# TopHillRobotics/quadruped-robot

Hardware: AMD Instinct MI355X
Metric: MPC+WBC control ticks/s (batched robots) (higher is better)
Workload: dtype f32 assembly / f64 QP+WBC

## Files before the change

### quadruped-robot_amd/csrc/qr_mpc_kernel.hip

```cpp
#include <hip/hip_runtime.h>
#include <type_traits>
#include "qr_device_types.h"
#include "qr_wave_helpers.h"
#include "qr_kernels.h"

namespace qrgpu {

#ifdef QR_TIMELINE
#define QR_TRACE(rid_, bits_) do { if (P.tl && P.solved) atomicOr((unsigned long long *)(P.tl + QR_TL_TRACE + (P.solved_epoch & 15u) * 1024 + ((rid_) & 1023)), (unsigned long long)(bits_) | ((unsigned long long)(P.solved_epoch & 15u) << 32) | (1ull << 40)); } while (0)
#define QR_P_TL P.tl
#define QR_P_FTIME P.ftime
#else
#define QR_TRACE(rid_, bits_) do { } while (0)
#define QR_P_TL ((long long *)nullptr)
#define QR_P_FTIME ((int *)nullptr)
#endif

#define QR_AS_THREADS 256
#define QR_RCP_PIVOT fast_rcp1
#define QR_REFRESH_EVERY 100
#ifdef QR_FLOPS_BUILD
#define qr_mpc_kernel qr_mpc_kernel_fl
#define mpc_solve_robot mpc_solve_robot_fl
#define QR_PFLOPS P.flops
// ... 487 lines not shown
                for (int r = r0; r < h; ++r) {
                    const bool onR = r >= iaR;
                    const float cR = ((float)r + bR) * dt2;
                    float gR = cR * a0R;
                    float tR = gR * w2q0;
                    gR = onR ? gR : 0.f; tR = onR ? tR : 0.f;
                    acc1 = __builtin_amdgcn_mfma_f32_16x16x4f32(tR, gR, acc1, 0, 0, 0);
                    const float hR = cR * a1R;
                    gR = (g < 2) ? hR : k1R; tR = (g < 2) ? hR * w2q1 : t1R;
                    gR = onR ? gR : 0.f; tR = onR ? tR : 0.f;
                    acc1 = __builtin_amdgcn_mfma_f32_16x16x4f32(tR, gR, acc1, 0, 0, 0);
                    gR = onR ? k2R : 0.f; tR = onR ? t2R : 0.f;
                    acc1 = __builtin_amdgcn_mfma_f32_16x16x4f32(tR, gR, acc1, 0, 0, 0);
                }
            } else {
                for (int r = r0; r < h; ++r) {
                    const bool onR = r >= iaR, onC = r >= iaC;
                    const float rf = (float)r;
                    const float cR = (rf + bR) * dt2, cC = (rf + bC) * dt2;
                    float gR = cR * a0R, gC = cC * a0C;
                    float tR = gR * w2q0, tC = gC * w2q0;
                    gR = onR ? gR : 0.f; tR = onR ? tR : 0.f; gC = onC ? gC : 0.f; tC = onC ? tC : 0.f;
                    acc1 = __builtin_amdgcn_mfma_f32_16x16x4f32(tR, gC, acc1, 0, 0, 0);
                    acc2 = __builtin_amdgcn_mfma_f32_16x16x4f32(gR, tC, acc2, 0, 0, 0);
                    const float hR = cR * a1R, hC = cC * a1C;
                    gR = (g < 2) ? hR : k1R; tR = (g < 2) ? hR * w2q1 : t1R;
                    gC = (g < 2) ? hC : k1C; tC = (g < 2) ? hC * w2q1 : t1C;
                    gR = onR ? gR : 0.f; tR = onR ? tR : 0.f; gC = onC ? gC : 0.f; tC = onC ? tC : 0.f;
                    acc1 = __builtin_amdgcn_mfma_f32_16x16x4f32(tR, gC, acc1, 0, 0, 0);
                    acc2 = __builtin_amdgcn_mfma_f32_16x16x4f32(gR, tC, acc2, 0, 0, 0);
                    gR = onR ? k2R : 0.f; tR = onR ? t2R : 0.f; gC = onC ? k2C : 0.f; tC = onC ? t2C : 0.f;
                    acc1 = __builtin_amdgcn_mfma_f32_16x16x4f32(tR, gC, acc1, 0, 0, 0);
                    acc2 = __builtin_amdgcn_mfma_f32_16x16x4f32(gR, tC, acc2, 0, 0, 0);
                }
            }
            float *buf = Hs + 256 * (diag ? 2 * NOD + R : 2 * (((R * (R - 1)) >> 1) + Cc));
#pragma unroll
            for (int reg = 0; reg < 4; ++reg) buf[((4 * reg + g) ^ (Cc & 1)) * 16 + lc] = acc1[reg];
            if (!diag) {
#pragma unroll
                for (int reg = 0; reg < 4; ++reg) buf[256 + ((4 * reg + g) ^ (Cc & 1)) * 16 + lc] = acc2[reg];
            }
            if (Hd) {
                const int ec = 16 * Cc + lc;
#pragma unroll
                for (int reg = 0; reg < 4; ++reg) {
                    const int er = 16 * R + 4 * g + reg;
                    if (er < ns && ec < ns) {
                        const int aq = (er * 21846) >> 16, bq = (ec * 21846) >> 16;
                        const int xr_ = 3 * sLs[aq] + (er - 3 * aq), xc_ = 3 * sLs[bq] + (ec - 3 * bq);
                        Hd[(size_t)xr_ * NV + xc_] = acc1[reg] + ((er == ec) ? two_alpha : 0.f);
                        if (!diag) Hd[(size_t)xc_ * NV + xr_] = acc2[reg];
                    }
                }
            }
          }
        }
    }
    for (int e = tid - (NTHR - 128); e >= 0 && e < ns; e += 128) {
#pragma clang fp contract(off)
        const int ls = sLs[e / 3], j = e % 3, ia = ls >> 2, p = ls & 3;
        const float t0 = sT[9 * p + j], t1 = sT[9 * p + 3 + j], t2 = sT[9 * p + 6 + j];
        const float wg0 = 2.f * C.weights[0], wg1 = 2.f * C.weights[1], wg2 = 2.f * C.weights[2], wg3 = 2.f * C.weights[3 + j], wg9 = 2.f * C.weights[9 + j];
        const float u0 = (dt * sU[9 * p + j]) * (2.f * C.weights[6]), u1 = (dt * sU[9 * p + 3 + j]) * (2.f * C.weights[7]), u2 = (dt * sU[9 * p + 6 + j]) * (2.f * C.weights[8]);
        const float dw = dtm * wg9;
        float acc = 0.f;
        const float bA = 0.5f - (float)ia;
        for (int r = 0; r < h; ++r) {
            const float ca = ((float)r + bA) * dt2;
            const float *vr = sV + 13 * r;
            float a2 = acc;
            a2 = __builtin_fmaf((ca * t0) * wg0, vr[0], a2);
            a2 = __builtin_fmaf((ca * t1) * wg1, vr[1], a2);
            a2 = __builtin_fmaf((ca * t2) * wg2, vr[2], a2);
            a2 = __builtin_fmaf((ca * minv) * wg3, vr[3 + j], a2);
            a2 = __builtin_fmaf(u0, vr[6], a2);
            a2 = __builtin_fmaf(u1, vr[7], a2);
            a2 = __builtin_fmaf(u2, vr[8], a2);
            a2 = __builtin_fmaf(dw, vr[9 + j], a2);
            acc = (r >= ia) ? a2 : acc;
        }
        gl[e] = (double)acc;
        if (QR_DBGG) QR_DBGG[(size_t)rid * NV + 3 * ls + j] = acc;
    }
    for (int c = tid; c < 6 * nls; c += NTHR) sPos[c] = -1;
    QR_TS(2);

    Blk A[MAXB];
    QR_SYNC();
#pragma unroll
    for (int sl = 0; sl < MAXB; ++sl) {
        if (ba[sl] >= 0) {
            const int a = ba[sl], b = bb[sl];
            int rowb[3], rr[3], rp[3], Rx[3], colb[3], cc[3], cp[3], Cy[3];
#pragma unroll
            for (int i = 0; i < 3; ++i) {
                const int x = 3 * a + i, y = 3 * b + i;
                Rx[i] = x >> 4; rr[i] = x & 15; rp[i] = 4 * (rr[i] & 3) + (rr[i] >> 2); rowb[i] = 256 * Rx[i] * (Rx[i] - 1);
                Cy[i] = y >> 4; cc[i] = y & 15; cp[i] = 4 * (cc[i] & 3) + (cc[i] >> 2); colb[i] = 512 * Cy[i] + cc[i];
            }
            const int dbase = 512 * NOD;
#pragma unroll
            for (int i = 0; i < 3; ++i)
#pragma unroll
                for (int j = 0; j < 3; ++j) {
                    if (a == b && j > i) continue;
                    const bool od = Rx[i] != Cy[j];
                    const int dg = dbase + 256 * Rx[i], par = Cy[j] & 1;
                    const int a1 = od ? rowb[i] + colb[j] + 16 * (rp[i] ^ par) : dg + 16 * (rp[i] ^ par) + cc[j];
                    const int a2 = od ? a1 + 256 : dg + 16 * (cp[j] ^ par) + rr[i];
                    float v1 = Hs[a1], v2 = Hs[a2];
                    if (a == b && i == j) {
#pragma clang fp contract(off)
                        v1 = v1 + two_alpha; v2 = v1;
                    }
                    const double o = 0.5 * ((double)v1 + (double)v2);
                    A[sl].m[3 * i + j] = o;
                    if (a == b) A[sl].m[3 * j + i] = o;
                }
        }
    }
    QR_SYNC();
    if (NTHR > QR_AS_THREADS && tid >= QR_AS_THREADS && (tid & ~63) >= npairs) { if (PERSIST) QR_IDLE(); return; }
    {
        double *panel0 = Mb, *panel1 = Mb + NL * 9;
#define VS_STAMP(i) do { } while (0)
        auto write_panel = [&](int sl, int kk, double *pn) {
            if (bb[sl] == kk) {
                if (ba[sl] == kk) {
                    const double *Pk = A[sl].m;
                    const double p00 = Pk[0], p01 = 0.5 * (Pk[1] + Pk[3]), p02 = 0.5 * (Pk[2] + Pk[6]), p11 = Pk[4], p12 = 0.5 * (Pk[5] + Pk[7]), p22 = Pk[8];
                    const double c00 = p11 * p22 - p12 * p12, c01 = p02 * p12 - p01 * p22, c02 = p01 * p12 - p02 * p11;
                    const double c11 = p00 * p22 - p02 * p02, c12 = p01 * p02 - p00 * p12, c22 = p00 * p11 - p01 * p01;
                    const double det = p00 * c00 + p01 * c01 + p02 * c02;
                    if (!(det > 0.0) || !(p00 > 0.0)) sMisc[1] = 1;
                    const double id = QR_RCP_PIVOT(det);
                    double *d = pn + 9 * kk;
                    d[0] = c00 * id; d[1] = c01 * id; d[2] = c02 * id; d[4] = c11 * id; d[5] = c12 * id; d[8] = c22 * id;
                } else {
#pragma unroll
                    for (int i = 0; i < 9; ++i) pn[9 * ba[sl] + i] = A[sl].m[i];
                }
            } else if (ba[sl] == kk) {
#pragma unroll
                for (int i = 0; i < 3; ++i)
#pragma unroll
                    for (int j = 0; j < 3; ++j) pn[9 * bb[sl] + 3 * j + i] = A[sl].m[3 * i + j];
            }
        };
#pragma unroll
        for (int sl = 0; sl < MAXB; ++sl) write_panel(sl, 0, panel0);
        for (int k = 0; k < nls; ++k) {
            double *pan = (k & 1) ? panel1 : panel0, *pnext = (k & 1) ? panel0 : panel1;
            VS_STAMP(3);
            VS_STAMP(0);
            QR_SYNC();
            VS_STAMP(1);
            double Cx0[9], Cb0[9];
            {
                const int a0 = ba[0] < 0 ? 0 : ba[0], b0 = ba[0] < 0 ? 0 : bb[0];
                const double *Cx = pan + 9 * (a0 == k ? b0 : a0), *Cb = pan + 9 * b0;
#pragma unroll
                for (int i = 0; i < 9; ++i) { Cx0[i] = Cx[i]; Cb0[i] = Cb[i]; }
            }
            double Pi[9];
            {
                const double *Pk = pan + 9 * k;
                Pi[0] = Pk[0]; Pi[1] = Pk[1]; Pi[2] = Pk[2]; Pi[4] = Pk[4]; Pi[5] = Pk[5]; Pi[8] = Pk[8];
                Pi[3] = Pi[1]; Pi[6] = Pi[2]; Pi[7] = Pi[5];
            }
            VS_STAMP(2);
#pragma unroll
            for (int sl = 0; sl < MAXB; ++sl) {
                const int a = ba[sl], b = bb[sl];
                if (a < 0) continue;
                double Cxv[9], Cb[9];
                if (sl == 0) {
#pragma unroll
                    for (int i = 0; i < 9; ++i) { Cxv[i] = Cx0[i]; Cb[i] = Cb0[i]; }
                } else {
                    const double *Cxp = pan + 9 * (a == k ? b : a), *Cbp = pan + 9 * b;
#pragma unroll
                    for (int i = 0; i < 9; ++i) { Cxv[i] = Cxp[i]; Cb[i] = Cbp[i]; }
                }
                const double *Cx = Cxv;
                double D[9];
#pragma unroll
                for (int i = 0; i < 3; ++i)
#pragma unroll
                    for (int j = 0; j < 3; ++j) D[3 * i + j] = __builtin_fma(Cx[3 * i + 2], Pi[6 + j], __builtin_fma(Cx[3 * i + 1], Pi[3 + j], Cx[3 * i] * Pi[j]));
                if (a != k && b != k) {
#pragma unroll
                    for (int i = 0; i < 3; ++i)
#pragma unroll
                        for (int j = 0; j < 3; ++j)
                            A[sl].m[3 * i + j] = __builtin_fma(-D[3 * i + 2], Cb[3 * j + 2], __builtin_fma(-D[3 * i + 1], Cb[3 * j + 1], __builtin_fma(-D[3 * i], Cb[3 * j], A[sl].m[3 * i + j])));
                } else {
                    const bool tr = (a == k);
                    A[sl].m[0] = D[0]; A[sl].m[4] = D[4]; A[sl].m[8] = D[8];
                    A[sl].m[1] = tr ? D[3] : D[1]; A[sl].m[3] = tr ? D[1] : D[3];
                    A[sl].m[2] = tr ? D[6] : D[2]; A[sl].m[6] = tr ? D[2] : D[6];
                    A[sl].m[5] = tr ? D[7] : D[5]; A[sl].m[7] = tr ? D[5] : D[7];
                    if (a == k && b == k) {
#pragma unroll
                        for (int i = 0; i < 9; ++i) A[sl].m[i] = -Pi[i];
                    }
                }
                write_panel(sl, k + 1, pnext);
                __builtin_amdgcn_sched_barrier(0);
            }
        }
        QR_SYNC();
#pragma unroll
        for (int sl = 0; sl < MAXB; ++sl) {
            if (ba[sl] >= 0) {
                double *dst = Mb + (tri(ba[sl]) + bb[sl]) * 9;
#pragma unroll
                for (int i = 0; i < 9; ++i) dst[i] = -A[sl].m[i];
            }
        }
        QR_SYNC();
    }
    if (NTHR > QR_AS_THREADS && tid >= QR_AS_THREADS) { if (PERSIST) QR_IDLE(); return; }
    if (sMisc[1]) st |= QRGPU_ST_MPC_NOTSPD;
    QR_TS(3);
    if (QR_PFLOPS) {
        double steps = 0.0;
        for (int Rf = 0; Rf < NT; ++Rf) steps += (double)(2 * Rf + 1) * (double)(h - (sLs[(16 * Rf * 21846) >> 16] >> 2));
        fl_m32 = steps * 3.0 * 2048.0;
        fl_v32 = steps * 64.0 * 8.0;
        double gsteps = 0.0;
        for (int kf = 0; kf < nls; ++kf) gsteps += (double)(h - (sLs[kf] >> 2));
        fl_v32 += gsteps * 3.0 * 24.0;
        fl_sw = (double)nls * ((double)npairs * 99.0 + 40.0) + (double)nls * (double)nls * 15.0;
    }
    {
        const int wv = __builtin_amdgcn_readfirstlane(tid >> 6);
        const bool own = lane < nls;
        const int kme = own ? lane : 0;
        const double im = (double)(1.f / C.mu);
        const double fmaxk = own ? fmk[kme] : 0.0;
        const int tril = tri(lane);
        const double tol = 1e-9;
        const double INF = __builtin_inf();
        const bool big2 = BIG && qcap > 64;
        double *xr2 = xr2_in_floats ? (double *)sT : smem + (P.lds_bytes / 8 - 256);
        const int tril2 = tri(lane + 64);
        auto rd2 = [&](double v0, double v1, int j) { return j < 64 ? readlane_d(v0, j) : readlane_d(v1, j - 64); };
        int *sCtl = sMisc + 8;
        double *dd = xz;
        enum { F_FULL = 1, F_DROP = 2 };
        double x0 = 0.0, x1 = 0.0, x2 = 0.0;
        {
            double p0 = 0.0, p1 = 0.0, p2 = 0.0;
            if (own) {
                for (int kc = wv; kc < nls; kc += 4) {
                    Blk B; load_block(Mb, kme, kc, B);
                    const double g0 = gl[3 * kc], g1 = gl[3 * kc + 1], g2 = gl[3 * kc + 2];
                    p0 += B.m[0] * g0 + B.m[1] * g1 + B.m[2] * g2;
                    p1 += B.m[3] * g0 + B.m[4] * g1 + B.m[5] * g2;
                    p2 += B.m[6] * g0 + B.m[7] * g1 + B.m[8] * g2;
                }
                xz[wv * NV + 3 * kme] = p0; xz[wv * NV + 3 * kme + 1] = p1; xz[wv * NV + 3 * kme + 2] = p2;
            }
            if (wv == 0) for (int e = lane; e < 6 * nls; e += 64) sPos[e] = (short)-1;
            QR_SYNC();
            if (own) {
#pragma unroll
                for (int v = 0; v < 4; ++v) { x0 -= xz[v * NV + 3 * kme]; x1 -= xz[v * NV + 3 * kme + 1]; x2 -= xz[v * NV + 3 * kme + 2]; }
                if (wv == 0) { gl[3 * kme] = x0; gl[3 * kme + 1] = x1; gl[3 * kme + 2] = x2; }
            }
            QR_SYNC();
        }
        QR_TS(4);
        bool fastz = qW > 0;
        auto r_partial = [&](int q, double dq, double dq2) {
            if (BIG && q > 64) {
                const int i1 = (lane + 64 < q) ? lane + 64 : 0;
                double pa = 0.0, pb = 0.0;
                for (int j = wv; j < q; j += 4) {
                    const double dj = rd2(dq, dq2, j);
                    pa += Sinv[(j <= lane) ? tril + j : tri(j) + lane] * dj;
                    pb += Sinv[(j <= i1) ? tri(i1) + j : tri(j) + i1] * dj;
                }
                xr[wv * 64 + lane] = pa; xr2[wv * 64 + lane] = pb;
                return;
            }
            const int i0 = (lane < q) ? lane : 0;
            double pr = 0.0;
            int j = wv;
            for (; j + 12 < q; j += 16) {
                double sv[4], dj[4];
#pragma unroll
                for (int u = 0; u < 4; ++u) { const int jj = j + 4 * u; sv[u] = Sinv[(jj <= i0) ? tril + jj : tri(jj) + i0]; dj[u] = readlane_d(dq, jj); }
#pragma unroll
                for (int u = 0; u < 4; ++u) pr += sv[u] * dj[u];
            }
            for (; j < q; j += 4) pr += Sinv[(j <= i0) ? tril + j : tri(j) + i0] * readlane_d(dq, j);
            xr[wv * 64 + lane] = pr;
        };
        auto rebuild = [&](const int q) -> bool {
            constexpr int NE = (QMAX * (QMAX + 1) / 2 + QR_AS_THREADS - 1) / QR_AS_THREADS;
            const int ne = tri(q);
            double *colp = xr;
            double *diag0 = xz + NV;
            constexpr int NER = (BIG && H16 && MAXB <= 4) ? 9 : NE;
            auto elem_ij = [&](const int e, int &i, int &j) {
                i = (int)((__builtin_sqrtf(8.f * (float)e + 1.f) - 1.f) * 0.5f);
                while (tri(i + 1) <= e) ++i;
                while (tri(i) > e) --i;
                j = e - tri(i);
            };
            double el[NER];
            int eij[NER];
            if constexpr (NER < NE) {
                for (int m = NER; QR_AS_THREADS * m < ne; ++m) {
                    const int e = tid + QR_AS_THREADS * m;
                    if (e < ne) {
                        int i, j; elem_ij(e, i, j);
                        const int ci = sAct[i], cj = sAct[j];
                        const int ki = (ci * 10923) >> 16, kj = (cj * 10923) >> 16;
                        Blk B; load_block(Mb, ki, kj, B);
                        double a0, a1, a2, b0, b1, b2;
                        cons_vec(ci - 6 * ki, im, a0, a1, a2); cons_vec(cj - 6 * kj, im, b0, b1, b2);
                        const double v = a0 * (B.m[0] * b0 + B.m[1] * b1 + B.m[2] * b2) + a1 * (B.m[3] * b0 + B.m[4] * b1 + B.m[5] * b2)
                                       + a2 * (B.m[6] * b0 + B.m[7] * b1 + B.m[8] * b2);
                        Sinv[e] = v;
                        if (j == 0) colp[i] = v;
                        if (i == j) diag0[i] = v;
                    }
                }
            }
#pragma unroll
            for (int m = 0; m < NER; ++m) {
                el[m] = 0.0; eij[m] = 0;
                if (QR_AS_THREADS * m < ne) {
                    int te = tid;
                    asm volatile("" : "+v"(te));
                    const int e = te + QR_AS_THREADS * m;
                    if (e < ne) {
                        int i = (int)((__builtin_sqrtf(8.f * (float)e + 1.f) - 1.f) * 0.5f);
                        while (tri(i + 1) <= e) ++i;
                        while (tri(i) > e) --i;
                        const int j = e - tri(i);
                        const int ci = sAct[i], cj = sAct[j];
                        const int ki = (ci * 10923) >> 16, kj = (cj * 10923) >> 16;
                        Blk B; load_block(Mb, ki, kj, B);
                        double a0, a1, a2, b0, b1, b2;
                        cons_vec(ci - 6 * ki, im, a0, a1, a2); cons_vec(cj - 6 * kj, im, b0, b1, b2);
                        const double v = a0 * (B.m[0] * b0 + B.m[1] * b1 + B.m[2] * b2) + a1 * (B.m[3] * b0 + B.m[4] * b1 + B.m[5] * b2)
                                       + a2 * (B.m[6] * b0 + B.m[7] * b1 + B.m[8] * b2);
                        el[m] = v; eij[m] = (i << 8) | j;
                        if (j == 0) colp[i] = v;
                        if (i == j) diag0[i] = v;
                    }
                }
            }
            QR_SYNC();
            bool ok = true;
            for (int p = 0; p < q; ++p) {
                const double *cur = colp + (p & 1) * QMAX;
                double *nxt = colp + ((p & 1) ^ 1) * QMAX;
                const double d = cur[p];
                if (!(d > 1e-11 * diag0[p])) { ok = false; break; }
                const double ip = QR_RCP_PIVOT(d);
                if constexpr (NER < NE) {
                    for (int m = NER; QR_AS_THREADS * m < ne; ++m) {
                        const int e = tid + QR_AS_THREADS * m;
                        if (e < ne) {
                            int i, j; elem_ij(e, i, j);
                            const double ci = cur[i], cj = cur[j];
                            const bool ip_ = (i == p), jp_ = (j == p);
                            const double sp_ = (ip_ && jp_) ? -ip : (ip_ ? cj : ci) * ip;
                            const double v = (ip_ || jp_) ? sp_ : Sinv[e] - ci * cj * ip;
                            Sinv[e] = v;
                            const bool c1 = (j == p + 1);
                            if (c1 || i == p + 1) nxt[c1 ? i : j] = v;
                        }
                    }
                }
#pragma unroll
                for (int m = 0; m < NER; ++m) {
                    if (QR_AS_THREADS * m < ne) {
                        const int i = eij[m] >> 8, j = eij[m] & 255;
                        const double ci = cur[i], cj = cur[j];
                        const bool ip_ = (i == p), jp_ = (j == p);
                        const double sp_ = (ip_ && jp_) ? -ip : (ip_ ? cj : ci) * ip;
                        const double v = (ip_ || jp_) ? sp_ : el[m] - ci * cj * ip;
                        el[m] = v;
                        const bool c1 = (j == p + 1);
                        if (c1 || i == p + 1) nxt[c1 ? i : j] = v;
                    }
                }
                QR_SYNC();
            }
            if (ok) {
#pragma unroll
                for (int m = 0; m < NER; ++m) { const int e = tid + QR_AS_THREADS * m; if (e < ne) Sinv[e] = -el[m]; }
                if constexpr (NER < NE) { for (int e = tid + QR_AS_THREADS * NER; e < ne; e += QR_AS_THREADS) Sinv[e] = -Sinv[e]; }
                if (qW > 0 && q <= qW) {
                    for (int i = wv; i < q; i += 4) {
                        const int ci = sAct[i];
                        const int ki = (ci * 10923) >> 16;
                        double a0, a1, a2;
                        cons_vec(ci - 6 * ki, im, a0, a1, a2);
                        if (own) {
                            Blk B; load_block(Mb, kme, ki, B);
                            double *wq = Wc + i * nsp + 3 * kme;
                            wq[0] = B.m[0] * a0 + B.m[1] * a1 + B.m[2] * a2;
                            wq[1] = B.m[3] * a0 + B.m[4] * a1 + B.m[5] * a2;
                            wq[2] = B.m[6] * a0 + B.m[7] * a1 + B.m[8] * a2;
                        }
                    }
                }
            }
            QR_SYNC();
            return ok;
        };
        enum { CMD_GO = 0, CMD_EXIT = 1, CMD_REBUILD = 2 };
        if (wv != 0) {
            const int g = wv - 1;
            for (;;) {
                QR_SYNC();
                const int cmd = __builtin_amdgcn_readfirstlane(sCtl[0]);
                if (cmd == CMD_EXIT) return;
                const int q = __builtin_amdgcn_readfirstlane(sCtl[1]);
                if (cmd == CMD_REBUILD) {
                    const bool ok = rebuild(q);
                    fastz = ok ? (qW > 0 && q <= qW) : (qW > 0);
                    continue;
                }
                const bool hi = BIG && q > 64;
                const double dq = (lane < q) ? dd[lane] : 0.0;
                const double dq2 = (hi && lane + 64 < q) ? dd[lane + 64] : 0.0;
                r_partial(q, dq, dq2);
                QR_SYNC();
                double rq, rq2 = 0.0;
                { const double rs = (xr[lane] + xr[64 + lane]) + (xr[128 + lane] + xr[192 + lane]); rq = (lane < q) ? rs : 0.0; }
                if (hi) { const double rs = (xr2[lane] + xr2[64 + lane]) + (xr2[128 + lane] + xr2[192 + lane]); rq2 = (lane + 64 < q) ? rs : 0.0; }
                double p0 = 0.0, p1 = 0.0, p2 = 0.0;
                if (fastz) {
                    const double *wk = Wc + 3 * kme;
                    int i = g;
                    for (; i + 3 < q; i += 6) {
                        const double ra = readlane_d(rq, i), rb = readlane_d(rq, i + 3);
                        const double *wa = wk + i * nsp, *wb = wk + (i + 3) * nsp;
                        const double a0 = wa[0], a1 = wa[1], a2 = wa[2], b0 = wb[0], b1 = wb[1], b2 = wb[2];
                        p0 += a0 * ra + b0 * rb; p1 += a1 * ra + b1 * rb; p2 += a2 * ra + b2 * rb;
                    }
                    if (i < q) { const double ra = readlane_d(rq, i); const double *wa = wk + i * nsp; p0 += wa[0] * ra; p1 += wa[1] * ra; p2 += wa[2] * ra; }
                } else if (q > 0) {
                    double y0 = 0.0, y1 = 0.0, y2 = 0.0;
                    bool hasrow = false;
#pragma unroll
                    for (int tq = 0; tq < 6; ++tq) {
                        const int ps = own ? (int)sPos[6 * kme + tq] : -1;
                        double rr = __shfl(rq, ps < 0 ? 0 : (ps & 63), 64);
                        if (hi) { const double r2 = __shfl(rq2, ps < 0 ? 0 : (ps & 63), 64); rr = ps >= 64 ? r2 : rr; }
                        if (ps >= 0) { double a0, a1, a2; cons_vec(tq, im, a0, a1, a2); y0 += a0 * rr; y1 += a1 * rr; y2 += a2 * rr; hasrow = true; }
                    }
                    const unsigned long long kall = __ballot(hasrow);
                    const int rank = __builtin_amdgcn_mbcnt_hi((unsigned)(kall >> 32), __builtin_amdgcn_mbcnt_lo((unsigned)kall, 0u));
                    const int r3 = rank - 3 * ((rank * 21846) >> 16);
                    unsigned long long km = __ballot(hasrow && r3 == g);
                    while (km) {
                        const int kc = (int)__builtin_ctzll(km);
                        km &= km - 1;
                        Blk B; load_block(Mb, kme, kc, B);
                        const double q0 = readlane_d(y0, kc), q1 = readlane_d(y1, kc), q2 = readlane_d(y2, kc);
                        p0 += B.m[0] * q0 + B.m[1] * q1 + B.m[2] * q2;
                        p1 += B.m[3] * q0 + B.m[4] * q1 + B.m[5] * q2;
                        p2 += B.m[6] * q0 + B.m[7] * q1 + B.m[8] * q2;
                    }
                }
                if (own) { xz[wv * NV + 3 * kme] = p0; xz[wv * NV + 3 * kme + 1] = p1; xz[wv * NV + 3 * kme + 2] = p2; }
                QR_SYNC();
                const int flags = __builtin_amdgcn_readfirstlane(sCtl[2]);
                if (flags & F_FULL) {
                    const double isg = __hiloint2double(__builtin_amdgcn_readfirstlane(sCtl[4]), __builtin_amdgcn_readfirstlane(sCtl[5]));
                    const bool act0 = lane < q;
                    const double ri = rq * isg;
                    int j = g;
                    if (hi) {
                        const bool act1 = lane + 64 < q;
                        const double ri2 = rq2 * isg;
                        for (; j < q; j += 3) {
                            const double rj = rd2(rq, rq2, j);
                            if (j <= lane) Sinv[tril + j] += ri * rj;
                            if (act1 && j <= lane + 64) Sinv[tril2 + j] += ri2 * rj;
                        }
                        if (g == 0) {
                            Sinv[tri(q) + lane] = -rq * isg;
                            if (act1) Sinv[tri(q) + 64 + lane] = -rq2 * isg;
                            if (lane == 0) Sinv[tri(q) + q] = isg;
                        }
                    } else {
                    for (; j + 9 < q; j += 12) {
                        double sv[4], rj[4];
#pragma unroll
                        for (int u = 0; u < 4; ++u) { const int jj = j + 3 * u; rj[u] = readlane_d(rq, jj); sv[u] = (act0 && jj <= lane) ? Sinv[tril + jj] : 0.0; }
#pragma unroll
                        for (int u = 0; u < 4; ++u) { const int jj = j + 3 * u; if (act0 && jj <= lane) Sinv[tril + jj] = sv[u] + ri * rj[u]; }
                    }
                    for (; j < q; j += 3) { const double rj = readlane_d(rq, j); if (act0 && j <= lane) Sinv[tril + j] += ri * rj; }
                    if (g == 0) {
                        if (act0) Sinv[tri(q) + lane] = -rq * isg;
                        if (lane == 0) Sinv[tri(q) + q] = isg;
                    }
                    }
                    if (fastz && !(q < qW)) fastz = false;
                } else if (flags & F_DROP) {
                    const int l = __builtin_amdgcn_readfirstlane(sCtl[3]), last = q - 1;
                    double sl = 0.0, sl2 = 0.0;
                    if (lane < q) sl = Sinv[pidx(lane, l)];
                    if (hi && lane + 64 < q) sl2 = Sinv[pidx(lane + 64, l)];
                    const double isl = fast_rcp(rd2(sl, sl2, l));
                    QR_SYNC();
                    for (int j = g; j < q; j += 3) {
                        if (j == l) continue;
                        const double sj = rd2(sl, sl2, j) * isl;
                        if (lane < q && lane != l && j <= lane) Sinv[tril + j] -= sl * sj;
                        if (hi && lane + 64 < q && lane + 64 != l && j <= lane + 64) Sinv[tril2 + j] -= sl2 * sj;
                    }
                    QR_SYNC();
                    double m0 = 0.0, m1 = 0.0;
                    if (l != last && g == 0 && lane < last) m0 = (lane == l) ? Sinv[tri(last) + last] : Sinv[pidx(last, lane)];
                    if (hi && l != last && g == 0 && lane + 64 < last) m1 = (lane + 64 == l) ? Sinv[tri(last) + last] : Sinv[pidx(last, lane + 64)];
                    QR_SYNC();
                    if (l != last && g == 0 && lane < last) Sinv[pidx(l, lane)] = m0;
                    if (hi && l != last && g == 0 && lane + 64 < last) Sinv[pidx(l, lane + 64)] = m1;
                }
            }
        }
        int q = 0, iter = 0;
#define CS_STAMP(i) do { } while (0)
#define CS_FINE(i) do { } while (0)
        unsigned amask = 0, xmask = 0;
        unsigned long long posk = 0;
        int ck = 0, ct = 0;
        double uq = 0.0;
        int ck2 = 0, ct2 = 0;
        double uq2 = 0.0;
        const int maxit = 40 * nls + 100;
        bool done = (nls == 0);
        bool need_rebuild = false;
        int refac = 0;
        int iter_at_rebuild = 0;
        unsigned char *warm = (P.warm && nls > 0) ? P.warm + (size_t)rid * QR_WARM_STRIDE : nullptr;
        const bool xtick = P.prev_solved != nullptr;
        bool warm_ok = true;
        long long t_waited = 0;
        if (xtick) {
            const long long c0_ = clock64();
            const long long t0 = wall_clock64();
            while (!qr_epoch_reached(__hip_atomic_load(P.prev_solved + rid, __ATOMIC_RELAXED, __HIP_MEMORY_SCOPE_AGENT), P.prev_epoch)) {
                if (wall_clock64() - t0 > P.xtick_wait) { st |= QRGPU_ST_PIPE_TIMEOUT; warm_ok = false; break; }
                __builtin_amdgcn_s_sleep(32);
            }
            t_waited = clock64() - c0_;
            if (lane == 0) QR_TRACE(rid, 32);
            if (lane == 0 && QR_P_TL) QR_P_TL[QR_TL_SOLVE_WAITS + (P.solved_epoch & 15u) * 1024 + (rid & 1023)] = ((wall_clock64() - t0) << 8) | (long long)(P.rescue_mode & 7) | (warm_ok ? 0 : 8);
        }
        auto warm_ld = [&](const unsigned char *p_) -> unsigned { return xtick ? (unsigned)__hip_atomic_load(p_, __ATOMIC_RELAXED, __HIP_MEMORY_SCOPE_AGENT) : (unsigned)*p_; };
        if (warm && warm_ok && warm_ld(warm + QR_WARM_STRIDE - 1) == (unsigned)(unsigned char)h) {
            const unsigned long long cur = ((unsigned long long)(unsigned)sMisc[3] << 32) | (unsigned)sMisc[2];
            const unsigned long long old = xtick ? __hip_atomic_load((const unsigned long long *)(warm + 64), __ATOMIC_RELAXED, __HIP_MEMORY_SCOPE_AGENT)
                                                 : *(const unsigned long long *)(warm + 64);
            int sh = 0, best = 1 << 30;
#pragma unroll
            for (int k = 0; k < 3; ++k) {
                const int keep = NL - 4 * k;
                const unsigned long long m = keep >= 64 ? ~0ull : ((1ull << keep) - 1ull);
                const int miss = __popcll(((old >> (4 * k)) ^ cur) & m) * 4 + k;
                if (miss < best) { best = miss; sh = k; }
            }
            const int src = own ? sLs[kme] + 4 * sh : NL;
            unsigned gm = (src < NL) ? warm_ld(warm + src) & 0x3fu : 0u;
            int base = 0;
            unsigned long long pk = 0;
#pragma unroll
            for (int t = 0; t < 6; ++t) {
                const bool has = (gm >> t) & 1u;
                const unsigned long long bal = __ballot(has);
                const int pos = base + __builtin_amdgcn_mbcnt_hi((unsigned)(bal >> 32), __builtin_amdgcn_mbcnt_lo((unsigned)bal, 0u));
                if (has && pos < 256) pk |= (unsigned long long)(pos & 0xff) << (8 * t);
                base += __popcll(bal);
            }
            const int qg = base;
            if (qg > 0 && qg <= qcap) {
                amask = gm; posk = pk; q = qg;
#pragma unroll
                for (int t = 0; t < 6; ++t)
                    if ((gm >> t) & 1u) { const int pos = (int)((pk >> (8 * t)) & 0xffu); sAct[pos] = 6 * kme + t; sPos[6 * kme + t] = (short)pos; }
                wave_sync();
                if (lane < q) { const int c = sAct[lane]; ck = (c * 10923) >> 16; ct = c - 6 * ck; }
                if (BIG && lane + 64 < q) { const int c = sAct[lane + 64]; ck2 = (c * 10923) >> 16; ct2 = c - 6 * ck2; }
                need_rebuild = true;
            }
        }
        auto slack_at_x0 = [&](int k_, int t_) {
            double a0, a1, a2;
            cons_vec(t_, im, a0, a1, a2);
            return a0 * gl[3 * k_] + a1 * gl[3 * k_ + 1] + a2 * gl[3 * k_ + 2] + ((t_ == 5) ? fmk[k_] : 0.0);
        };
        while (!done) {
            if (need_rebuild) {
                need_rebuild = false;
                xmask = 0;
                if (lane < q) sAct[lane] = 6 * ck + ct;
                if (BIG && lane + 64 < q) sAct[lane + 64] = 6 * ck2 + ct2;
                if (lane == 0) { sCtl[0] = CMD_REBUILD; sCtl[1] = q; }
                QR_SYNC();
                const bool ok = rebuild(q);
                if (QR_PFLOPS) fl_as += 17.5 * (double)q * (double)q + 1.5 * (double)q * (double)q * (double)q + 15.0 * (double)q * (double)nls;
                if (!ok) {
                    if (own) {
#pragma unroll
                        for (int t = 0; t < 6; ++t) sPos[6 * kme + t] = (short)-1;
                    }
                    amask = 0; posk = 0; q = 0; uq = 0.0; uq2 = 0.0;
                    x0 = gl[3 * kme]; x1 = gl[3 * kme + 1]; x2 = gl[3 * kme + 2];
                    fastz = qW > 0;
                    refac = 2;
                    continue;
                }
                fastz = qW > 0 && q <= qW;
                for (;;) {
                    if (++iter > maxit) { st |= QRGPU_ST_MPC_MAXITER; done = true; break; }
                    q = __builtin_amdgcn_readfirstlane(q);
                    const bool hi = BIG && q > 64;
                    const double dq = (lane < q) ? slack_at_x0(ck, ct) : 0.0;
                    double dq2 = 0.0;
                    if (hi) { dq2 = (lane + 64 < q) ? slack_at_x0(ck2, ct2) : 0.0; if (lane + 64 < q) dd[lane + 64] = dq2; }
                    if (lane < q) dd[lane] = dq;
                    if (lane == 0) { sCtl[0] = CMD_GO; sCtl[1] = q; }
                    QR_SYNC();
                    r_partial(q, dq, dq2);
                    QR_SYNC();
                    double rq, rq2 = 0.0;
                    { const double rs = (xr[lane] + xr[64 + lane]) + (xr[128 + lane] + xr[192 + lane]); rq = (lane < q) ? rs : 0.0; }
                    if (hi) { const double rs = (xr2[lane] + xr2[64 + lane]) + (xr2[128 + lane] + xr2[192 + lane]); rq2 = (lane + 64 < q) ? rs : 0.0; }
                    if (QR_PFLOPS) fl_as += 3.0 * (double)q * (double)q + 6.0 * (double)nls * (double)q + 8.0 * (double)q;
                    const double umax = -wave_min_d(hi ? (rq < rq2 ? rq : rq2) : rq);
                    const double worst = -wave_min_d(hi ? (-rq < -rq2 ? -rq : -rq2) : -rq);
                    const bool drop = worst > 1e-10 * (1.0 + (umax > 0.0 ? umax : 0.0));
                    const double thr_neg = 1e-10 * (1.0 + (umax > 0.0 ? umax : 0.0));
                    const bool neg1 = lane < q && rq > thr_neg, neg2 = hi && lane + 64 < q && rq2 > thr_neg;
                    const int nneg = __popcll(__ballot(neg1)) + (hi ? __popcll(__ballot(neg2)) : 0);
                    const bool block_drop = drop && P.no_block_drop != 1 && nneg >= (P.no_block_drop > 1 ? (P.no_block_drop >> 8) : 4) && (P.no_block_drop > 1 ? (P.no_block_drop & 255) : 4) * nneg >= q && nneg < q;
                    int lpos = -1;
                    if (drop && !block_drop) { lpos = first_lane(lane < q && rq == worst); if (hi && lpos < 0) lpos = 64 + first_lane(lane + 64 < q && rq2 == worst); }
                    if (lane == 0) { sCtl[2] = (drop && !block_drop) ? F_DROP : 0; sCtl[3] = lpos; }
                    QR_SYNC();
                    if (block_drop) {
                        const unsigned long long k1 = __ballot(lane < q && !neg1), k2 = hi ? __ballot(lane + 64 < q && !neg2) : 0ull;
                        const int n1 = __popcll(k1);
                        const int np1 = __builtin_amdgcn_mbcnt_hi((unsigned)(k1 >> 32), __builtin_amdgcn_mbcnt_lo((unsigned)k1, 0u));
                        const int np2 = n1 + __builtin_amdgcn_mbcnt_hi((unsigned)(k2 >> 32), __builtin_amdgcn_mbcnt_lo((unsigned)k2, 0u));
                        if (own) {
#pragma unroll
                            for (int t = 0; t < 6; ++t) sPos[6 * kme + t] = (short)-1;
                        }
                        wave_sync();
                        if (lane < q && !neg1) { sAct[np1] = 6 * ck + ct; sPos[6 * ck + ct] = (short)np1; }
                        if (hi && lane + 64 < q && !neg2) { sAct[np2] = 6 * ck2 + ct2; sPos[6 * ck2 + ct2] = (short)np2; }
                        q = n1 + (hi ? __popcll(k2) : 0);
                        wave_sync();
                        if (lane < q) { const int c = sAct[lane]; ck = (c * 10923) >> 16; ct = c - 6 * ck; }
                        if (BIG && lane + 64 < q) { const int c = sAct[lane + 64]; ck2 = (c * 10923) >> 16; ct2 = c - 6 * ck2; }
                        amask = 0; posk = 0;
                        if (own) {
#pragma unroll
                            for (int t = 0; t < 6; ++t) { const int ps = sPos[6 * kme + t]; if (ps >= 0) { amask |= 1u << t; posk |= (unsigned long long)(ps & 0xff) << (8 * t); } }
                        }
                        need_rebuild = true;
                        break;
                    }
                    if (!drop) {
                        x0 = gl[3 * kme] - ((xz[NV + 3 * kme] + xz[2 * NV + 3 * kme]) + xz[3 * NV + 3 * kme]);
                        x1 = gl[3 * kme + 1] - ((xz[NV + 3 * kme + 1] + xz[2 * NV + 3 * kme + 1]) + xz[3 * NV + 3 * kme + 1]);
                        x2 = gl[3 * kme + 2] - ((xz[NV + 3 * kme + 2] + xz[2 * NV + 3 * kme + 2]) + xz[3 * NV + 3 * kme + 2]);
                        uq = (lane < q && rq < 0.0) ? -rq : 0.0;
                        if (hi) uq2 = (lane + 64 < q && rq2 < 0.0) ? -rq2 : 0.0;
                        break;
                    }
                    {
                        const int l = lpos, last = q - 1;
                        int clk, clt, cmk, cmt;
                        if (BIG && l >= 64) { clk = __builtin_amdgcn_readlane(ck2, l - 64); clt = __builtin_amdgcn_readlane(ct2, l - 64); }
                        else { clk = __builtin_amdgcn_readlane(ck, l); clt = __builtin_amdgcn_readlane(ct, l); }
                        if (BIG && last >= 64) { cmk = __builtin_amdgcn_readlane(ck2, last - 64); cmt = __builtin_amdgcn_readlane(ct2, last - 64); }
                        else { cmk = __builtin_amdgcn_readlane(ck, last); cmt = __builtin_amdgcn_readlane(ct, last); }
                        QR_SYNC();
                        if (fastz && l != last && own) { const double *wl_ = Wc + last * nsp + 3 * kme; double *wd_ = Wc + l * nsp + 3 * kme; wd_[0] = wl_[0]; wd_[1] = wl_[1]; wd_[2] = wl_[2]; }
                        QR_SYNC();
                        if (l != last) {
                            if (lane == l) { ck = cmk; ct = cmt; }
                            if (BIG && lane + 64 == l) { ck2 = cmk; ct2 = cmt; }
                        }
                        if (lane == clk) { amask &= ~(1u << clt); sPos[6 * clk + clt] = (short)-1; }
                        if (l != last && lane == cmk) { posk = (posk & ~(0xffull << (8 * cmt))) | ((unsigned long long)l << (8 * cmt)); sPos[6 * cmk + cmt] = (short)l; }
                        QR_SYNC();
                        --q;
                    }
                    if (q == 0) { x0 = gl[3 * kme]; x1 = gl[3 * kme + 1]; x2 = gl[3 * kme + 2]; uq = 0.0; uq2 = 0.0; break; }
                }
                if (done) break;
                if (need_rebuild) continue;
            }
            CS_FINE(1);
            double bs = INF; int bt = 0;
            {
                const double s[6] = {im * x0 + x2, -im * x0 + x2, im * x1 + x2, -im * x1 + x2, x2, fmaxk - x2};
                const unsigned blocked = own ? (amask | xmask) : 0x3fu;
#pragma unroll
                for (int t = 0; t < 6; ++t) { const bool take = !((blocked >> t) & 1u) && s[t] < bs; bs = take ? s[t] : bs; bt = take ? t : bt; }
            }
            CS_FINE(2);
            const double smin = wave_min_d(bs);
            CS_FINE(3);
            if (!(smin < -tol)) {
                double be = 0.0;
                if (own && (xmask | amask)) {
                    const double s[6] = {im * x0 + x2, -im * x0 + x2, im * x1 + x2, -im * x1 + x2, x2, fmaxk - x2};
#pragma unroll
                    for (int t = 0; t < 6; ++t) {
                        if (((xmask >> t) & 1u) && s[t] < be) be = s[t];
                        if (((amask >> t) & 1u) && -__builtin_fabs(s[t]) < be) be = -__builtin_fabs(s[t]);
                    }
                }
                const double bemin = wave_min_d(be);
                if (bemin < -1e-4) {
                    if (refac < 2 && q > 0) { ++refac; need_rebuild = true; continue; }
                    st |= QRGPU_ST_MPC_INFEAS;
                }
                break;
            }
            if (iter - iter_at_rebuild >= QR_REFRESH_EVERY && q > 0) { iter_at_rebuild = iter; need_rebuild = true; continue; }
            const int kp = __builtin_amdgcn_readfirstlane(first_lane(bs == smin));
            const int tp = __builtin_amdgcn_readlane(bt, kp);
            double c0, c1, c2;
            cons_vec(tp, im, c0, c1, c2);
            const double ci0p = (tp == 5) ? readlane_d(fmaxk, kp) : 0.0;
            double up = 0.0;
            CS_STAMP(0);
            for (;;) {
                q = __builtin_amdgcn_readfirstlane(q);
                if (++iter > maxit) { st |= QRGPU_ST_MPC_MAXITER; done = true; break; }
                double w0, w1, w2_;
                {
                    Blk B; load_block(Mb, kme, kp, B);
                    w0 = B.m[0] * c0 + B.m[1] * c1 + B.m[2] * c2;
                    w1 = B.m[3] * c0 + B.m[4] * c1 + B.m[5] * c2;
                    w2_ = B.m[6] * c0 + B.m[7] * c1 + B.m[8] * c2;
                }
                const double delta = c0 * readlane_d(w0, kp) + c1 * readlane_d(w1, kp) + c2 * readlane_d(w2_, kp);
                double dq;
                {
                    double a0, a1, a2;
                    cons_vec(ct, im, a0, a1, a2);
                    const double g0 = __shfl(w0, ck, 64), g1 = __shfl(w1, ck, 64), g2 = __shfl(w2_, ck, 64);
                    dq = (lane < q) ? a0 * g0 + a1 * g1 + a2 * g2 : 0.0;
                }
                const bool hi = BIG && q > 64;
                double dq2 = 0.0;
                if (hi) {
                    double a0, a1, a2;
                    cons_vec(ct2, im, a0, a1, a2);
                    const double g0 = __shfl(w0, ck2, 64), g1 = __shfl(w1, ck2, 64), g2 = __shfl(w2_, ck2, 64);
                    dq2 = (lane + 64 < q) ? a0 * g0 + a1 * g1 + a2 * g2 : 0.0;
                    if (lane + 64 < q) dd[lane + 64] = dq2;
                }
                if (lane < q) dd[lane] = dq;
                if (lane == 0) { sCtl[0] = 0; sCtl[1] = q; }
                CS_STAMP(1);
                QR_SYNC();
                CS_STAMP(2);
                r_partial(q, dq, dq2);
                QR_SYNC();
                CS_STAMP(3);
                double rq, rq2 = 0.0;
                { const double rs = (xr[lane] + xr[64 + lane]) + (xr[128 + lane] + xr[192 + lane]); rq = (lane < q) ? rs : 0.0; }
                if (hi) { const double rs = (xr2[lane] + xr2[64 + lane]) + (xr2[128 + lane] + xr2[192 + lane]); rq2 = (lane + 64 < q) ? rs : 0.0; }
                const double dr = wave_sum_d(hi ? rq * dq + rq2 * dq2 : rq * dq);
                const double zc = delta - dr;
                double tt, tt2 = INF;
                { const double tq_ = uq * fast_rcp(rq); tt = (lane < q && rq > 0.0) ? tq_ : INF; }
                if (hi) { const double tq_ = uq2 * fast_rcp(rq2); tt2 = (lane + 64 < q && rq2 > 0.0) ? tq_ : INF; }
                const double t1 = wave_min_d(hi ? (tt < tt2 ? tt : tt2) : tt);
                int lpos = (t1 < INF) ? first_lane(tt == t1) : -1;
                if (hi && t1 < INF && lpos < 0) lpos = 64 + first_lane(tt2 == t1);
                const double sp = c0 * readlane_d(x0, kp) + c1 * readlane_d(x1, kp) + c2 * readlane_d(x2, kp) + ci0p;
                const bool have_z = zc > 1e-13 * delta;
                const bool indep = zc > 1e-9 * delta;
                const double izc = fast_rcp(zc);
                const double t2 = indep ? -sp * izc : INF;
                const double t = t1 < t2 ? t1 : t2;
                const bool degenerate = !(t < INF);
                const bool full = !degenerate && indep && t == t2;
                const bool over = full && q >= qcap;
                const int flags = (degenerate || over) ? 0 : (full ? F_FULL : F_DROP);
                if (lane == 0) { sCtl[2] = flags; sCtl[3] = lpos; sCtl[4] = __double2hiint(izc); sCtl[5] = __double2loint(izc); }
                CS_STAMP(4);
                QR_SYNC();
                CS_STAMP(5);
                if (degenerate) { if (lane == kp) xmask |= 1u << tp; break; }
                if (over) { st |= QRGPU_ST_MPC_OVERFLOW; done = true; break; }
                if (have_z) {
                    const double z0 = w0 - ((xz[NV + 3 * kme] + xz[2 * NV + 3 * kme]) + xz[3 * NV + 3 * kme]);
                    const double z1 = w1 - ((xz[NV + 3 * kme + 1] + xz[2 * NV + 3 * kme + 1]) + xz[3 * NV + 3 * kme + 1]);
                    const double z2 = w2_ - ((xz[NV + 3 * kme + 2] + xz[2 * NV + 3 * kme + 2]) + xz[3 * NV + 3 * kme + 2]);
                    x0 += t * z0; x1 += t * z1; x2 += t * z2;
                }
                uq -= t * rq;
                if (hi) uq2 -= t * rq2;
                up += t;
                CS_FINE(0);
                if (QR_PFLOPS) fl_as += 3.0 * (double)q * (double)q + 6.0 * (double)nls * (double)q + 21.0 * (double)nls + 12.0 * (double)q;
                if (full) {
                    if (fastz) {
                        if (q < qW) { if (own) { int kl = lane; asm volatile("" : "+v"(kl)); double *wq = Wc + q * nsp + 3 * kl; wq[0] = w0; wq[1] = w1; wq[2] = w2_; } }
                        else fastz = false;
                    }
                    if (lane == q) { uq = up; ck = kp; ct = tp; }
                    if (BIG && lane + 64 == q) { uq2 = up; ck2 = kp; ct2 = tp; }
                    if (lane == kp) { amask |= 1u << tp; posk = (posk & ~(0xffull << (8 * tp))) | ((unsigned long long)q << (8 * tp)); sPos[6 * kp + tp] = (short)q; }
                    xmask = 0;
                    ++q;
                    break;
                }
                {
                    const int l = lpos, last = q - 1;
                    int clk, clt, cmk, cmt;
                    double ulast;
                    if (BIG && l >= 64) { clk = __builtin_amdgcn_readlane(ck2, l - 64); clt = __builtin_amdgcn_readlane(ct2, l - 64); }
                    else { clk = __builtin_amdgcn_readlane(ck, l); clt = __builtin_amdgcn_readlane(ct, l); }
                    if (BIG && last >= 64) { cmk = __builtin_amdgcn_readlane(ck2, last - 64); cmt = __builtin_amdgcn_readlane(ct2, last - 64); ulast = readlane_d(uq2, last - 64); }
                    else { cmk = __builtin_amdgcn_readlane(ck, last); cmt = __builtin_amdgcn_readlane(ct, last); ulast = readlane_d(uq, last); }
                    QR_SYNC();
                    if (fastz && l != last && own) { const double *wl_ = Wc + last * nsp + 3 * kme; double *wd_ = Wc + l * nsp + 3 * kme; wd_[0] = wl_[0]; wd_[1] = wl_[1]; wd_[2] = wl_[2]; }
                    QR_SYNC();
                    if (l != last) {
                        if (lane == l) { uq = ulast; ck = cmk; ct = cmt; }
                        if (BIG && lane + 64 == l) { uq2 = ulast; ck2 = cmk; ct2 = cmt; }
                    }
                    if (lane == clk) { amask &= ~(1u << clt); sPos[6 * clk + clt] = (short)-1; }
                    if (l != last && lane == cmk) { posk = (posk & ~(0xffull << (8 * cmt))) | ((unsigned long long)l << (8 * cmt)); sPos[6 * cmk + cmt] = (short)l; }
                    QR_SYNC();
                    xmask = 0;
                    --q;
                }
            }
        }
        if (lane == 0) { sCtl[0] = CMD_EXIT; sMisc[15] = nbar + 1; }
        QR_SYNC();
        QR_TS(5);
        const bool to_rescue = (st & QRGPU_ST_MPC_OVERFLOW) && P.rescue_list && !P.rescue_mode;
        if (warm && !to_rescue) {
            const bool good = (st & 0xff) == 0;
            auto warm_st = [&](unsigned char *p_, unsigned char v_) { if (P.solved) __hip_atomic_store(p_, v_, __ATOMIC_RELAXED, __HIP_MEMORY_SCOPE_AGENT); else *p_ = v_; };
            warm_st(warm + lane, 0);
            wave_sync();
            unsigned keep = amask;
            if (P.warm_uthr > 0.0) {
                const double um = -wave_min_d((lane < q) ? -uq : 0.0);
                const double um2 = (BIG && q > 64) ? -wave_min_d((lane + 64 < q) ? -uq2 : 0.0) : 0.0;
                const double thr_u = P.warm_uthr * (um > um2 ? um : um2);
#pragma unroll
                for (int t = 0; t < 6; ++t) {
                    const int pos = (int)((posk >> (8 * t)) & 0xffu);
                    const double ut = (BIG && pos >= 64) ? __shfl(uq2, pos - 64, 64) : __shfl(uq, pos & 63, 64);
                    if (((amask >> t) & 1u) && !(ut > thr_u)) keep &= ~(1u << t);
                }
            }
            if (own && good) warm_st(warm + sLs[kme], (unsigned char)keep);
            if (lane == 0) {
                const unsigned long long tbl = ((unsigned long long)(unsigned)sMisc[3] << 32) | (unsigned)sMisc[2];
                if (P.solved) __hip_atomic_store((unsigned long long *)(warm + 64), tbl, __ATOMIC_RELAXED, __HIP_MEMORY_SCOPE_AGENT);
                else *(unsigned long long *)(warm + 64) = tbl;
                warm_st(warm + QR_WARM_STRIDE - 1, good ? (unsigned char)h : (unsigned char)0);
            }
        }
        wave_sync();
        if (lane < 12) xz[lane] = 0.0;
        wave_sync();
        if (own) { const int ls = sLs[kme]; if (ls < 4) { xz[3 * ls] = x0; xz[3 * ls + 1] = x1; xz[3 * ls + 2] = x2; } }
        wave_sync();
        {
            float Ro[3][3];
            const float *qs = (const float *)sMisc + 4;
            quat_to_rot(qs[0], qs[1], qs[2], qs[3], Ro);
            mpc_outputs(lane, rid, n, xz, Ro, sJ, C, io.g_q, io.g_force, io.g_force_wbc, io.force_stride, io.g_tau, P.epilogue, P.done_flag != nullptr);
        }
        if (lane == 0 && io.g_status) {
            if (P.done_flag) __hip_atomic_store(io.g_status + rid, st | ((iter & 0xffff) << 8), __ATOMIC_RELAXED, __HIP_MEMORY_SCOPE_AGENT);
            else io.g_status[rid] = st | ((iter & 0xffff) << 8);
        }
        if (to_rescue && P.main_done) asm volatile("s_waitcnt vmcnt(0)" ::: "memory");
        if (lane == 0 && to_rescue) QR_TRACE(rid, 64);
        if (lane == 0 && to_rescue) st_through(P.rescue_list + atomicAdd(P.rescue_count + P.rescue_parity, 1), rid, P.solved != nullptr);
        if (P.done_flag) {
            asm volatile("s_waitcnt vmcnt(0)" ::: "memory");
            if (lane == 0) {
                const unsigned mine = (P.done_epoch << 1) | (to_rescue ? 1u : 0u);
                unsigned cur = __hip_atomic_load(P.done_flag + rid, __ATOMIC_RELAXED, __HIP_MEMORY_SCOPE_AGENT);
                bool late = false;
                for (int tries = 0; tries < 64; ++tries) {
                    const unsigned ce = (cur >> 1) & 0x3fffffffu;
                    late = cur == (0x80000000u | (P.done_epoch << 1));
                    if (ce != P.done_epoch && qr_epoch_reached(ce, P.done_epoch)) { late = true; break; }
                    const unsigned seen = atomicCAS(P.done_flag + rid, cur, mine);
                    if (seen == cur) break;
                    cur = seen;
                }
                if (late && io.g_status) __hip_atomic_fetch_or(io.g_status + rid, QRGPU_ST_PIPE_TIMEOUT, __ATOMIC_RELAXED, __HIP_MEMORY_SCOPE_AGENT);
            }
            if (lane == 0 && QR_P_FTIME) QR_P_FTIME[rid] = (int)wall_clock64();
// ... 342 lines not shown
```

Baseline: 4.507 million.

## Block active-set inverse rebuild into 2x2 pivot steps and interleave W fill

The active-set Schur-complement inverse rebuild now eliminates two pivots per step using an explicit 2x2 block inverse, with interleaved two-column buffers. This halves the number of block-wide barriers in the rebuild loop. The W-column fill is spread across the pivot groups instead of running as a separate pass afterwards. The cost is more arithmetic per element per step and a more complex pivot check, which can change numerical behaviour near singular pivots.

```diff
diff --git a/quadruped-robot_amd/csrc/qr_mpc_kernel.hip b/quadruped-robot_amd/csrc/qr_mpc_kernel.hip
--- a/quadruped-robot_amd/csrc/qr_mpc_kernel.hip
+++ b/quadruped-robot_amd/csrc/qr_mpc_kernel.hip
@@ -813,7 +813,8 @@
         auto rebuild = [&](const int q) -> bool {
             constexpr int NE = (QMAX * (QMAX + 1) / 2 + QR_AS_THREADS - 1) / QR_AS_THREADS;
             const int ne = tri(q);
-            double *colp = xr;
+            double *colA = xr, *colB = xz + 2 * NV;
+                        auto uni = [](double v) { return __hiloint2double(__builtin_amdgcn_readfirstlane(__double2hiint(v)), __builtin_amdgcn_readfirstlane(__double2loint(v))); };
             double *diag0 = xz + NV;
             constexpr int NER = (BIG && H16 && MAXB <= 4) ? 9 : NE;
             auto elem_ij = [&](const int e, int &i, int &j) {
@@ -837,7 +838,8 @@
                         const double v = a0 * (B.m[0] * b0 + B.m[1] * b1 + B.m[2] * b2) + a1 * (B.m[3] * b0 + B.m[4] * b1 + B.m[5] * b2)
                                        + a2 * (B.m[6] * b0 + B.m[7] * b1 + B.m[8] * b2);
                         Sinv[e] = v;
-                        if (j == 0) colp[i] = v;
+                        if (j < 2) colA[2 * i + j] = v;
+                        if (i == 1) colA[2 * j + 1] = v;
                         if (i == j) diag0[i] = v;
                     }
                 }
@@ -862,55 +864,35 @@
                         const double v = a0 * (B.m[0] * b0 + B.m[1] * b1 + B.m[2] * b2) + a1 * (B.m[3] * b0 + B.m[4] * b1 + B.m[5] * b2)
                                        + a2 * (B.m[6] * b0 + B.m[7] * b1 + B.m[8] * b2);
                         el[m] = v; eij[m] = (i << 8) | j;
-                        if (j == 0) colp[i] = v;
+                        if (j < 2) colA[2 * i + j] = v;
+                        if (i == 1) colA[2 * j + 1] = v;
                         if (i == j) diag0[i] = v;
                     }
                 }
             }
+            if (q == 1 && tid == 0) colA[1] = 0.0;
             QR_SYNC();
             bool ok = true;
-            for (int p = 0; p < q; ++p) {
-                const double *cur = colp + (p & 1) * QMAX;
-                double *nxt = colp + ((p & 1) ^ 1) * QMAX;
-                const double d = cur[p];
-                if (!(d > 1e-11 * diag0[p])) { ok = false; break; }
-                const double ip = QR_RCP_PIVOT(d);
-                if constexpr (NER < NE) {
-                    for (int m = NER; QR_AS_THREADS * m < ne; ++m) {
-                        const int e = tid + QR_AS_THREADS * m;
-                        if (e < ne) {
-                            int i, j; elem_ij(e, i, j);
-                            const double ci = cur[i], cj = cur[j];
-                            const bool ip_ = (i == p), jp_ = (j == p);
-                            const double sp_ = (ip_ && jp_) ? -ip : (ip_ ? cj : ci) * ip;
-                            const double v = (ip_ || jp_) ? sp_ : Sinv[e] - ci * cj * ip;
-                            Sinv[e] = v;
-                            const bool c1 = (j == p + 1);
-                            if (c1 || i == p + 1) nxt[c1 ? i : j] = v;
-                        }
-                    }
-                }
-#pragma unroll
-                for (int m = 0; m < NER; ++m) {
-                    if (QR_AS_THREADS * m < ne) {
-                        const int i = eij[m] >> 8, j = eij[m] & 255;
-                        const double ci = cur[i], cj = cur[j];
-                        const bool ip_ = (i == p), jp_ = (j == p);
-                        const double sp_ = (ip_ && jp_) ? -ip : (ip_ ? cj : ci) * ip;
-                        const double v = (ip_ || jp_) ? sp_ : el[m] - ci * cj * ip;
-                        el[m] = v;
-                        const bool c1 = (j == p + 1);
-                        if (c1 || i == p + 1) nxt[c1 ? i : j] = v;
-                    }
-                }
-                QR_SYNC();
-            }
-            if (ok) {
-#pragma unroll
-                for (int m = 0; m < NER; ++m) { const int e = tid + QR_AS_THREADS * m; if (e < ne) Sinv[e] = -el[m]; }
-                if constexpr (NER < NE) { for (int e = tid + QR_AS_THREADS * NER; e < ne; e += QR_AS_THREADS) Sinv[e] = -Sinv[e]; }
-                if (qW > 0 && q <= qW) {
-                    for (int i = wv; i < q; i += 4) {
+            const bool fillW = qW > 0 && q <= qW;
+            for (int p = 0, grp = 0; p < q; p += 2, ++grp) {
+                const double *cur = (grp & 1) ? colB : colA;
+                double *nxt = (grp & 1) ? colA : colB;
+                const bool two = p + 1 < q;
+                const double a = uni(cur[2 * p]);
+                const double b = two ? uni(cur[2 * p + 1]) : 0.0;
+                const double c = two ? uni(cur[2 * p + 3]) : 1.0;
+                const double d2 = c - b * b * QR_RCP_PIVOT(a);
+                if (!(a > 1e-11 * uni(diag0[p])) || (two && !(d2 > 1e-11 * uni(diag0[p + 1])))) { ok = false; break; }
+                const double idet = QR_RCP_PIVOT(a * c - b * b);
+                const double I00 = c * idet, I01 = -b * idet, I11 = a * idet;
+#if QR_X_FILL == 0
+                if (fillW) {
+                    const int i = 4 * grp + wv;
+                    if (i < q) {
+#else
+                }}};
+                auto fill_row = [&](const int i) {{{
+#endif
                         const int ci = sAct[i];
                         const int ki = (ci * 10923) >> 16;
                         double a0, a1, a2;
@@ -924,6 +906,47 @@
                         }
                     }
                 }
+#if QR_X_FILL != 0
+            if (0) { if (0) { if (0) {
+#endif
+                auto upd = [&](const int i, const int j, const double old) -> double {
+                    const double ai = cur[2 * i], bi = cur[2 * i + 1], aj = cur[2 * j], bj = cur[2 * j + 1];
+                    const int di = i - p, dj = j - p;
+                    const bool iP = (unsigned)di < 2u, jP = (unsigned)dj < 2u;
+                    const double xa = iP ? aj : ai, xb = iP ? bj : bi;
+                    const double ua = I00 * xa + I01 * xb, ub = I01 * xa + I11 * xb;
+                    const double vP = (iP ? di : dj) ? ub : ua;
+                    const double vPP = -(di == 0 ? I00 : (dj == 0 ? I01 : I11));
+                    const double v = (iP && jP) ? vPP : ((iP || jP) ? vP : old - (ua * aj + ub * bj));
+                    const int ni = di - 2, nj = dj - 2;
+                    if ((unsigned)nj < 2u) nxt[2 * i + nj] = v;
+                    if ((unsigned)ni < 2u) nxt[2 * j + ni] = v;
+                    return v;
+                };
+                if constexpr (NER < NE) {
+                    for (int m = NER; QR_AS_THREADS * m < ne; ++m) {
+                        const int e = tid + QR_AS_THREADS * m;
+                        if (e < ne) {
+                            int i, j; elem_ij(e, i, j);
+                            Sinv[e] = upd(i, j, Sinv[e]);
+                        }
+                    }
+                }
+#pragma unroll
+                for (int m = 0; m < NER; ++m) {
+                    if (QR_AS_THREADS * m < ne) {
+                        int ev = eij[m];
+                        asm volatile("" : "+v"(ev));
+                        el[m] = upd(ev >> 8, ev & 255, el[m]);
+                    }
+                }
+                if (p + 3 == q && tid < q) nxt[2 * tid + 1] = 0.0;
+                QR_SYNC();
+            }
+            if (ok) {
+#pragma unroll
+                for (int m = 0; m < NER; ++m) { const int e = tid + QR_AS_THREADS * m; if (e < ne) Sinv[e] = -el[m]; }
+                if constexpr (NER < NE) { for (int e = tid + QR_AS_THREADS * NER; e < ne; e += QR_AS_THREADS) Sinv[e] = -Sinv[e]; }
             }
             QR_SYNC();
             return ok;
@@ -1123,7 +1146,7 @@
                 if (lane == 0) { sCtl[0] = CMD_REBUILD; sCtl[1] = q; }
                 QR_SYNC();
                 const bool ok = rebuild(q);
-                if (QR_PFLOPS) fl_as += 17.5 * (double)q * (double)q + 1.5 * (double)q * (double)q * (double)q + 15.0 * (double)q * (double)nls;
+                if (QR_PFLOPS) fl_as += 17.5 * (double)q * (double)q + 2.5 * (double)q * (double)q * (double)q + 15.0 * (double)q * (double)nls;
                 if (!ok) {
                     if (own) {
 #pragma unroll
```

Measured after the change: 4.500 million. No clear change (-0.2%).
